# annikabrundyn/driving-dirty

Measured on AMD Instinct MI355X. Metric: 6-view scenes/sec fwd+bwd, roadmap model bs=32, higher is better.
Workload: dtype f32

## Files before the change

driving-dirty_amd/csrc/conv3x3.hip:

```cpp
#include <stdlib.h>

#include "dd_common.h"

namespace {

constexpr int EPI_BIAS_RELU_BITS = 5;
constexpr int EPI_RELU_BITS = 6;
constexpr int EPI_BIAS_STATS = 7;
constexpr int EPI_RELU_MASK_AFF = 8;
constexpr int EPI_RELU_BITS_W1 = 9;


template <int CIN, int S>
struct StripCfg {
  static constexpr int PXB = CIN * 4;
  static constexpr int CHUNKS = CIN / 4;
  static constexpr int NPX = 32 * S + 2;
  static constexpr int SLOTB = NPX * PXB;
  static constexpr int NCH = NPX * CHUNKS;
  static constexpr int NLOAD = (NCH + 63) / 64;
  static constexpr int SPILLB = (NLOAD * 64 - NCH) * 16;
  static constexpr int WAVEB = 3 * SLOTB + SPILLB;
  static constexpr int KGROUPS = (CIN == 32) ? 36 : 5;
  static constexpr int WFLOATS = KGROUPS * 64 * 4;
// ... 66 lines not shown
    v.z = in ? fmaxf(v.z * sc.z + sh.z, 0.f) : 0.f;
    v.w = in ? fmaxf(v.w * sc.w + sh.w, 0.f) : 0.f;
    *(f32x4*)dst = v;
  }
}

template <int CIN, int S, int EPI, int WPB, bool AFF = false>
__global__ __launch_bounds__(WPB * 64) void conv_strip_fwd(const float* __restrict__ x, const float* __restrict__ wp,
                                                           const float* __restrict__ bias,
                                                           const float* __restrict__ msk, float* __restrict__ y,
                                                           unsigned* __restrict__ bits_out, int B, int H, int W, int Ho,
                                                           int Wo, int nstrips, const float* __restrict__ aff = nullptr,
                                                           float* __restrict__ stats = nullptr) {
  using C = StripCfg<CIN, S>;
  extern __shared__ __attribute__((aligned(16))) char smem[];
  const int tid = threadIdx.x;
  const int lane = tid & 63;
  const int wave = __builtin_amdgcn_readfirstlane(tid >> 6);
  {
    f32x4* wl4 = (f32x4*)smem;
    const f32x4* wg4 = (const f32x4*)wp;
    for (int i = tid; i < C::WFLOATS / 4; i += WPB * 64) wl4[i] = wg4[i];
  }
  __syncthreads();
  char* ring = smem + C::WFLOATS * 4 + wave * C::WAVEB;
  char* spill = ring + 3 * C::SLOTB;
  const char* wl = smem;
  const int h = lane >> 5, n = lane & 31;
  const float bv = (EPI == DD_EPI_BIAS || EPI == DD_EPI_BIAS_RELU || EPI == EPI_BIAS_RELU_BITS || EPI == EPI_BIAS_STATS) ? bias[n] : 0.f;
  f32x4 asc = {1.f, 1.f, 1.f, 1.f}, ash = {0.f, 0.f, 0.f, 0.f};
  if (AFF) {
    asc = *(const f32x4*)(aff + 4 * (lane & 7));
    ash = *(const f32x4*)(aff + 32 + 4 * (lane & 7));
  }
  const float msc = (EPI == EPI_RELU_MASK_AFF) ? aff[64 + n] : 1.f, msh = (EPI == EPI_RELU_MASK_AFF) ? aff[96 + n] : 0.f;
  float st_sum = 0.f, st_sq = 0.f;

  long idx, end;
  dd_range((long)B * nstrips * Ho, blockIdx.x * WPB + wave, gridDim.x * WPB, idx, end);
  while (idx < end) {
    const long col = idx / Ho;
    const int y0 = (int)(idx - col * Ho);
    const int y1 = (int)min((long)Ho, y0 + (end - idx));
    idx += y1 - y0;
    const int b = (int)(col / nstrips), x0 = (int)(col % nstrips) * 32;
    const float* xb = x + (long)b * H * W * CIN;
    const int gx0 = S * x0 - 1;

#pragma unroll
    for (int d = 0; d < 3; ++d) {
      f32x4 t[C::NLOAD];
      const int iy = S * y0 - 1 + d;
      load_row<CIN, S>(xb, H, W, iy, gx0, lane, t);
      if constexpr (AFF) store_row_aff<S, true>(ring + ((iy + 1) % 3) * C::SLOTB, spill, lane, t, iy >= 0 && iy < H, gx0, W, asc, ash);
      else store_row<CIN, S, true>(ring + ((iy + 1) % 3) * C::SLOTB, spill, lane, t);
    }

    for (int yy = y0; yy < y1; ++yy) {
      f32x4 pre[S][C::NLOAD];
#pragma unroll
      for (int s = 0; s < S; ++s) load_row<CIN, S>(xb, H, W, S * yy + 2 + s, gx0, lane, pre[s]);

      const long orow = ((long)(b * Ho + yy) * Wo) * 32;
      float mreg[16];
      if (EPI == DD_EPI_RELU_MASK || EPI == EPI_RELU_MASK_AFF) {
        const __amdgpu_buffer_rsrc_t ms = dd_rsrc(msk + orow, Wo * 128);
#pragma unroll
        for (int r = 0; r < 16; ++r) mreg[r] = dd_bload1<DD_AUX_NT>(ms, ((x0 + dd_acc_row(r, lane)) * 32 + n) * 4);
      }
      if (EPI == EPI_RELU_BITS) {
        const __amdgpu_buffer_rsrc_t ms = dd_rsrc((const unsigned*)msk + (long)(b * Ho + yy) * Wo, Wo * 4);
#pragma unroll
        for (int r = 0; r < 16; ++r) mreg[r] = dd_bload1<DD_AUX_NT>(ms, (x0 + dd_acc_row(r, lane)) * 4);
      }
      __builtin_amdgcn_sched_barrier(0);

      f32x16 acc;
#pragma unroll
      for (int r = 0; r < 16; ++r) acc[r] = 0.f;

      if (CIN == 32) {
#pragma unroll
        for (int dy = 0; dy < 3; ++dy) {
          const char* rowb = ring + ((S * yy + dy) % 3) * C::SLOTB;
#pragma unroll
          for (int dx = 0; dx < 3; ++dx) {
            const int q = S * n + dx;
            const char* pa = rowb + q * 128;
            const int sw = swz<32>(q);
#pragma unroll
            for (int j = 0; j < 4; ++j) {
              const f32x4 a = *(const f32x4*)(pa + (((2 * j + h) ^ sw) << 4));
              const f32x4 w = *(const f32x4*)(wl + (((dy * 3 + dx) * 4 + j) * 64 + lane) * 16);
              acc = DD_MFMA(a.x, w.x, acc);
              acc = DD_MFMA(a.y, w.y, acc);
              acc = DD_MFMA(a.z, w.z, acc);
              acc = DD_MFMA(a.w, w.w, acc);
            }
          }
        }
      } else {
#pragma unroll
        for (int jp = 0; jp < 5; ++jp) {
          const int tap = min(2 * jp + h, 8);
          const int dy = tap / 3, dx = tap - 3 * dy;
          const char* rowb = ring + ((S * yy + dy) % 3) * C::SLOTB;
          const f32x4 a = *(const f32x4*)(rowb + (S * n + dx) * 16);
          const f32x4 w = *(const f32x4*)(wl + (jp * 64 + lane) * 16);
          acc = DD_MFMA(a.x, w.x, acc);
          acc = DD_MFMA(a.y, w.y, acc);
          acc = DD_MFMA(a.z, w.z, acc);
        }
      }

#pragma unroll
      for (int s = 0; s < S; ++s) {
        const int iy = S * yy + 2 + s;
        if constexpr (AFF) store_row_aff<S, true>(ring + ((iy + 1) % 3) * C::SLOTB, spill, lane, pre[s], iy >= 0 && iy < H, gx0, W, asc, ash);
        else store_row<CIN, S, true>(ring + ((iy + 1) % 3) * C::SLOTB, spill, lane, pre[s]);
      }

      const __amdgpu_buffer_rsrc_t ys = dd_rsrc(y + orow, Wo * 128);
      unsigned sign_word = 0;
#pragma unroll
      for (int r = 0; r < 16; ++r) {
        float v = acc[r];
        if (EPI == DD_EPI_BIAS || EPI == EPI_BIAS_STATS) v += bv;
        if (EPI == EPI_BIAS_STATS && x0 + dd_acc_row(r, lane) < Wo) {
          st_sum += v;
          st_sq += v * v;
        }
        if (EPI == DD_EPI_BIAS_RELU || EPI == EPI_BIAS_RELU_BITS) v = fmaxf(v + bv, 0.f);
        if (EPI == DD_EPI_RELU_MASK) v = (mreg[r] > 0.f) ? v : 0.f;
        if (EPI == EPI_RELU_MASK_AFF) v = (mreg[r] * msc + msh > 0.f) ? v : 0.f;
        if (EPI == EPI_RELU_BITS) v = ((__builtin_bit_cast(unsigned, mreg[r]) >> n) & 1u) ? v : 0.f;
        dd_bstore1<DD_AUX_NT>(ys, ((x0 + dd_acc_row(r, lane)) * 32 + n) * 4, v);
        if (EPI == EPI_BIAS_RELU_BITS) {
          const unsigned long long m = __ballot(v > 0.f);
          const int i0 = (r & 3) + 8 * (r >> 2);
          if (n == i0) sign_word = (unsigned)m;
          if (n == i0 + 4) sign_word = (unsigned)(m >> 32);
        }
      }
      if (EPI == EPI_BIAS_RELU_BITS) {
        const __amdgpu_buffer_rsrc_t bs = dd_rsrc(bits_out + (long)(b * Ho + yy) * Wo, Wo * 4);
        __builtin_amdgcn_raw_buffer_store_b32(sign_word, bs, (h == 0) ? (x0 + n) * 4 : -16, 0, 0);
      }
    }
  }
  if (EPI == EPI_BIAS_STATS) {
    const long gwl = ((long)(blockIdx.x * WPB + wave) * 64 + lane) * 2;
    stats[gwl] = st_sum;
    stats[gwl + 1] = st_sq;
  }
}

template <int WPB, int MASK>
__global__ __launch_bounds__(WPB * 64) void conv_s2_dgrad(const float* __restrict__ dy, const float* __restrict__ wp,
                                                          const float* __restrict__ msk, float* __restrict__ dx,
                                                          int B, int H, int W, int Ho, int Wo, int nstrips,
                                                          const float* __restrict__ aff = nullptr) {
  using C = StripCfg<32, 1>;
  extern __shared__ __attribute__((aligned(16))) char smem[];
  const int tid = threadIdx.x;
  const int lane = tid & 63;
  const int wave = __builtin_amdgcn_readfirstlane(tid >> 6);
  {
    f32x4* wl4 = (f32x4*)smem;
    const f32x4* wg4 = (const f32x4*)wp;
    for (int i = tid; i < C::WFLOATS / 4; i += WPB * 64) wl4[i] = wg4[i];
  }
  __syncthreads();
  const int nr = (H + 1) / 2;
  const float msc = (MASK == 3) ? aff[64 + (lane & 31)] : 1.f, msh = (MASK == 3) ? aff[96 + (lane & 31)] : 0.f;
  char* ring = smem + C::WFLOATS * 4 + wave * C::WAVEB;
  char* spill = ring + 3 * C::SLOTB;
  const char* wl = smem;
  const int h = lane >> 5, n = lane & 31;

  long idx, end;
  dd_range((long)B * nstrips * nr, blockIdx.x * WPB + wave, gridDim.x * WPB, idx, end);
  while (idx < end) {
    const long col = idx / nr;
    const int r0 = (int)(idx - col * nr);
    const int r1 = (int)min((long)nr, r0 + (end - idx));
    idx += r1 - r0;
    const int b = (int)(col / nstrips), s0 = (int)(col % nstrips) * 32;
    const float* dyb = dy + (long)b * Ho * Wo * 32;

#pragma unroll
    for (int d = 0; d < 2; ++d) {
      f32x4 t[C::NLOAD];
      load_row<32, 1>(dyb, Ho, Wo, r0 + d, s0, lane, t);
      store_row<32, 1, true>(ring + ((r0 + d) % 3) * C::SLOTB, spill, lane, t);
    }

    for (int r = r0; r < r1; ++r) {
      f32x4 pre[C::NLOAD];
      load_row<32, 1>(dyb, Ho, Wo, r + 2, s0, lane, pre);
      __builtin_amdgcn_sched_barrier(0);

      const char* row_r = ring + (r % 3) * C::SLOTB;
      const char* row_r1 = ring + ((r + 1) % 3) * C::SLOTB;
#define DD_TILE(PY, PX, NTAP, ...)                                                              \
  {                                                                                             \
    constexpr int taps[NTAP][3] = {__VA_ARGS__};                                                \
    const int yi = 2 * r + (PY);                                                                \
    const long orow = ((long)(b * H + min(yi, H - 1)) * W) * 32;                                \
    const int obytes = (yi < H) ? W * 128 : 0;                                                  \
    float mreg[16];                                                                             \
    if (MASK == 1 || MASK == 3) {                                                               \
      const __amdgpu_buffer_rsrc_t ms = dd_rsrc(msk + orow, obytes);                            \
      _Pragma("unroll") for (int rr = 0; rr < 16; ++rr)                                         \
        mreg[rr] = dd_bload1<DD_AUX_NT>(ms, ((2 * (s0 + dd_acc_row(rr, lane)) + (PX)) * 32 + n) * 4); \
      __builtin_amdgcn_sched_barrier(0);                                                        \
    }                                                                                           \
    if (MASK == 2) {                                                                            \
      const __amdgpu_buffer_rsrc_t ms = dd_rsrc((const unsigned*)msk + (long)(b * H + min(yi, H - 1)) * W, obytes / 32); \
      _Pragma("unroll") for (int rr = 0; rr < 16; ++rr)                                         \
        mreg[rr] = dd_bload1<DD_AUX_NT>(ms, (2 * (s0 + dd_acc_row(rr, lane)) + (PX)) * 4);      \
      __builtin_amdgcn_sched_barrier(0);                                                        \
    }                                                                                           \
    f32x16 acc;                                                                                 \
    _Pragma("unroll") for (int i = 0; i < 16; ++i) acc[i] = 0.f;                                \
    _Pragma("unroll") for (int t = 0; t < NTAP; ++t) {                                          \
      const char* rowp = taps[t][0] ? row_r1 : row_r;                                           \
      const int q = n + taps[t][1];                                                             \
      const char* pa = rowp + q * 128;                                                          \
      const int sw = swz<32>(q);                                                                \
      _Pragma("unroll") for (int j = 0; j < 4; ++j) {                                           \
        const f32x4 a = *(const f32x4*)(pa + (((2 * j + h) ^ sw) << 4));                        \
        const f32x4 w = *(const f32x4*)(wl + ((taps[t][2] * 4 + j) * 64 + lane) * 16);          \
        acc = DD_MFMA(a.x, w.x, acc);                                                           \
        acc = DD_MFMA(a.y, w.y, acc);                                                           \
        acc = DD_MFMA(a.z, w.z, acc);                                                           \
        acc = DD_MFMA(a.w, w.w, acc);                                                           \
      }                                                                                         \
    }                                                                                           \
    const __amdgpu_buffer_rsrc_t os = dd_rsrc(dx + orow, obytes);                               \
    _Pragma("unroll") for (int rr = 0; rr < 16; ++rr) {                                         \
      float v = acc[rr];                                                                        \
      if (MASK == 1) v = (mreg[rr] > 0.f) ? v : 0.f;                                            \
      if (MASK == 3) v = (mreg[rr] * msc + msh > 0.f) ? v : 0.f;                                \
      if (MASK == 2) v = ((__builtin_bit_cast(unsigned, mreg[rr]) >> n) & 1u) ? v : 0.f;        \
      dd_bstore1<DD_AUX_NT>(os, ((2 * (s0 + dd_acc_row(rr, lane)) + (PX)) * 32 + n) * 4, v);    \
    }                                                                                           \
  }
      DD_TILE(1, 1, 4, {1, 1, 0}, {1, 0, 2}, {0, 1, 6}, {0, 0, 8})
      store_row<32, 1, true>(ring + ((r + 2) % 3) * C::SLOTB, spill, lane, pre);
      DD_TILE(0, 1, 2, {0, 1, 3}, {0, 0, 5})
      DD_TILE(1, 0, 2, {1, 0, 1}, {0, 0, 7})
      DD_TILE(0, 0, 1, {0, 0, 4})
#undef DD_TILE
    }
  }
}

template <int CIN, int S, int WPB, bool AFF = false>
__global__ __launch_bounds__(WPB * 64) void conv_wgrad(const float* __restrict__ x, const float* __restrict__ dy,
                                                       float* __restrict__ part, float* __restrict__ bpart, int B,
                                                       int H, int W, int Ho, int Wo, int nstrips,
                                                       const float* __restrict__ aff = nullptr) {
  using C = StripCfg<CIN, S>;
  constexpr int NT = (CIN == 32) ? 9 : 1;
  extern __shared__ __attribute__((aligned(16))) char smem[];
  const int tid = threadIdx.x;
  const int lane = tid & 63;
  const int wave = __builtin_amdgcn_readfirstlane(tid >> 6);
  char* ring = smem + wave * C::WAVEB;
  char* spill = ring + 3 * C::SLOTB;
  const int h = lane >> 5, n = lane & 31;
  const int gw = blockIdx.x * WPB + wave;
  f32x4 asc = {1.f, 1.f, 1.f, 1.f}, ash = {0.f, 0.f, 0.f, 0.f};
  if (AFF) {
    asc = *(const f32x4*)(aff + 4 * (lane & 7));
    ash = *(const f32x4*)(aff + 32 + 4 * (lane & 7));
  }

  f32x16 acc[NT];
#pragma unroll
  for (int t = 0; t < NT; ++t)
#pragma unroll
    for (int r = 0; r < 16; ++r) acc[t][r] = 0.f;
  float bsum = 0.f;

  const int tap4 = min(n / 3, 8), c4 = n % 3;
  const int dy4 = tap4 / 3, dx4 = tap4 - 3 * dy4;

  long idx, end;
  dd_range((long)B * nstrips * Ho, gw, gridDim.x * WPB, idx, end);
  while (idx < end) {
    const long col = idx / Ho;
    const int y0 = (int)(idx - col * Ho);
    const int y1 = (int)min((long)Ho, y0 + (end - idx));
    idx += y1 - y0;
    const int b = (int)(col / nstrips), x0 = (int)(col % nstrips) * 32;
    const float* xb = x + (long)b * H * W * CIN;
    const float* dyb = dy + (long)b * Ho * Wo * 32;
    const int gx0 = S * x0 - 1;
    const int aoff = ((x0 + h) * 32 + n) * 4;

#pragma unroll
    for (int d = 0; d < 3; ++d) {
      f32x4 t[C::NLOAD];
      const int iy = S * y0 - 1 + d;
      load_row<CIN, S>(xb, H, W, iy, gx0, lane, t);
// ... 1342 lines not shown
      for (int c = 0; c < W2R_CHUNKS; ++c) t += tv[u][c];
      t = t * ((u == 1 || u == 2) ? 0.5f : 1.f) * ((v == 1 || v == 2) ? 0.5f : 1.f);
      z[0] += (u < 3 ? 1.f : 0.f) * t;
      z[1] += (u == 1 ? 1.f : u == 2 ? -1.f : 0.f) * t;
      z[2] += (u > 0 ? 1.f : 0.f) * t;
    }
#pragma unroll
    for (int ky = 0; ky < 3; ++ky) {
      out[ky][0] += (v < 3 ? 1.f : 0.f) * z[ky];
      out[ky][1] += (v == 1 ? 1.f : v == 2 ? -1.f : 0.f) * z[ky];
      out[ky][2] += (v > 0 ? 1.f : 0.f) * z[ky];
    }
  }
  const int o = dd_acc_row(r, l), jj = l & 31;
  float* dst = dw + ((long)o * 32 + jj) * 9;
#pragma unroll
  for (int a = 0; a < 9; ++a) dst[a] = out[a / 3][a % 3];
}

__global__ __launch_bounds__(1024) void conv_wino_wgrad_reduce(const float* __restrict__ part, const float* __restrict__ bpart,
                                                               float* __restrict__ dw, float* __restrict__ db, int nw) {
  constexpr int G = 16;
  __shared__ float red[4][G][64];
  const int l = threadIdx.x & 63, g = threadIdx.x >> 6;
  const int row = blockIdx.x;
  if (row == 48) {
    float s0 = 0.f;
    for (int w = g; w < nw; w += G) s0 += bpart[(long)w * 64 + l];
    red[0][g][l] = s0;
    __syncthreads();
    if (g != 0) return;
    float s = 0.f;
#pragma unroll
    for (int i = 0; i < G; ++i) s += red[0][i][l];
    const float other = __shfl_xor(s, 32);
    if (l < 32) db[l] = s + other;
    return;
  }
  const int ky = row >> 4, r = row & 15;
  float s[4] = {0.f, 0.f, 0.f, 0.f};
  for (int w = g; w < nw; w += G) {
#pragma unroll
    for (int p = 0; p < 4; ++p) s[p] += part[((((long)w * 3 + ky) * 4 + p) * 16 + r) * 64 + l];
  }
#pragma unroll
  for (int p = 0; p < 4; ++p) red[p][g][l] = s[p];
  __syncthreads();
  if (g != 0) return;
  float t[4] = {0.f, 0.f, 0.f, 0.f};
#pragma unroll
  for (int p = 0; p < 4; ++p)
#pragma unroll
    for (int i = 0; i < G; ++i) t[p] += red[p][i][l];
  const int o = dd_acc_row(r, l), j = l & 31;
  float* out = dw + ((long)o * 32 + j) * 9 + ky * 3;
  out[0] = (t[0] + t[1]) + t[2];
  out[1] = t[1] - t[2];
  out[2] = (t[1] + t[2]) + t[3];
}

__global__ void conv_wino_pack_kernel(const float* __restrict__ w, float* __restrict__ p, int kind) {
  const int idx = blockIdx.x * blockDim.x + threadIdx.x;
  if (idx >= WINO_UFLOATS) return;
  const int j = idx & 3, lane = (idx >> 2) & 63, g = (idx >> 8) & 1, hf = (idx >> 9) & 1, pos = (idx >> 10) & 3, ky = idx >> 12;
  const int co = (lane & 15) + 16 * hf, ci = 8 * (lane >> 4) + 4 * g + j;
  float t[3];
#pragma unroll
  for (int kx = 0; kx < 3; ++kx)
    t[kx] = kind == 0 ? w[((long)co * 32 + ci) * 9 + ky * 3 + kx] : w[((long)ci * 32 + co) * 9 + (2 - ky) * 3 + (2 - kx)];
  float u;
  if (pos == 0) u = t[0];
  else if (pos == 1) u = 0.5f * ((t[0] + t[1]) + t[2]);
  else if (pos == 2) u = 0.5f * ((t[0] - t[1]) + t[2]);
  else u = t[2];
  p[idx] = u;
}

__global__ __launch_bounds__(256) void relu_sign_bits_kernel(const float* __restrict__ x, unsigned* __restrict__ bits, long npix) {
  const int lane = threadIdx.x & 63;
  const long wave = ((long)blockIdx.x * blockDim.x + threadIdx.x) >> 6, nwaves = ((long)gridDim.x * blockDim.x) >> 6;
  for (long p0 = wave * 64; p0 < npix; p0 += nwaves * 64) {
    unsigned word = 0;
#pragma unroll 8
    for (int i = 0; i < 32; ++i) {
      const long p = p0 + 2 * i + (lane >> 5);
      const float v = p < npix ? x[p * 32 + (lane & 31)] : 0.f;
      const unsigned long long m = __ballot(v > 0.f);
      if (lane == 2 * i) word = (unsigned)m;
      if (lane == 2 * i + 1) word = (unsigned)(m >> 32);
    }
    if (p0 + lane < npix) bits[p0 + lane] = word;
  }
}

__global__ __launch_bounds__(256) void relu_bwd_pad_bits_kernel(const float* __restrict__ dy, const unsigned* __restrict__ bits_pad,
                                                                f32x4* __restrict__ out_pad, int B, int H, int W, int dy_cstore, int dy_coff) {
  const long total = (long)B * (H + 2) * (W + 2) * 8;
  for (long i = (long)blockIdx.x * blockDim.x + threadIdx.x; i < total; i += (long)gridDim.x * blockDim.x) {
    const int q = (int)(i & 7);
    const long pp = i >> 3;
    const int xx = (int)(pp % (W + 2)), yy = (int)((pp / (W + 2)) % (H + 2));
    const long b = pp / ((long)(W + 2) * (H + 2));
    f32x4 o = {0.f, 0.f, 0.f, 0.f};
    if (xx >= 1 && xx <= W && yy >= 1 && yy <= H) {
      const f32x4 g = *(const f32x4*)(dy + ((b * H + (yy - 1)) * W + (xx - 1)) * dy_cstore + dy_coff + 4 * q);
      const unsigned m = bits_pad[pp] >> (4 * q);
      o.x = (m & 1u) ? g.x : 0.f;
      o.y = (m & 2u) ? g.y : 0.f;
      o.z = (m & 4u) ? g.z : 0.f;
      o.w = (m & 8u) ? g.w : 0.f;
    }
    __builtin_nontemporal_store(o, out_pad + i);
  }
}

__global__ void relu_bwd_kernel(const f32x4* __restrict__ dy, const f32x4* __restrict__ y, f32x4* __restrict__ out,
                                long n4) {
  for (long i = (long)blockIdx.x * blockDim.x + threadIdx.x; i < n4; i += (long)gridDim.x * blockDim.x) {
    const f32x4 g = dy[i], v = y[i];
    f32x4 o;
    o.x = v.x > 0.f ? g.x : 0.f;
    o.y = v.y > 0.f ? g.y : 0.f;
    o.z = v.z > 0.f ? g.z : 0.f;
    o.w = v.w > 0.f ? g.w : 0.f;
    out[i] = o;
  }
}

int check_desc(const dd_conv_desc* d) {
  DD_REQUIRE(d != nullptr, DD_ERR_BAD_ARG, "conv: NULL descriptor");
  DD_REQUIRE(d->batch > 0 && d->height > 0 && d->width > 0, DD_ERR_BAD_ARG, "conv: non-positive size");
  DD_REQUIRE(d->ksize == 3 && d->pad == 1, DD_ERR_UNSUPPORTED, "conv: only k3 p1 is implemented (got k%d p%d)", d->ksize, d->pad);
  DD_REQUIRE(d->stride == 1 || d->stride == 2, DD_ERR_UNSUPPORTED, "conv: stride %d", d->stride);
  DD_REQUIRE(d->cout == 32, DD_ERR_UNSUPPORTED, "conv: Cout %d (only 32)", d->cout);
  DD_REQUIRE((d->cin_real == 32 && d->cin_store == 32) || (d->cin_real == 3 && d->cin_store == 4), DD_ERR_UNSUPPORTED,
             "conv: Cin %d stored as %d (supported: 32/32, 3/4)", d->cin_real, d->cin_store);
  DD_REQUIRE(!(d->cin_real == 3 && d->stride == 2), DD_ERR_UNSUPPORTED, "conv: Cin 3 with stride 2");
  DD_REQUIRE((long)d->width * 128 < (1L << 31), DD_ERR_UNSUPPORTED, "conv: row too long for a 32-bit buffer descriptor");
  return 0;
}

int resident_grid(const dd_conv_desc* d, long row_tiles, int wpb, int per_cu) {
  long blocks = (long)dd_cu_budget_internal() * per_cu;
  if (d->rows_per_task > 0) blocks = min(blocks, max(1L, row_tiles / d->rows_per_task / wpb));
  return (int)max(1L, min(blocks, (row_tiles + wpb - 1) / wpb));
}

template <int CIN, int S, int EPI, int WPB, bool AFF = false>
int launch_fwd(const float* x, const float* wp, const float* bias, const float* msk, float* y, const dd_conv_desc* d,
               hipStream_t st, unsigned* bits_out = nullptr, const float* aff = nullptr, float* stats = nullptr) {
  using C = StripCfg<CIN, S>;
  const int Ho = dd_conv_out(d->height, S), Wo = dd_conv_out(d->width, S);
  const int nstrips = (Wo + 31) / 32;
  const size_t lds = C::WFLOATS * 4 + (size_t)WPB * C::WAVEB;
  const int per_cu = (int)max((size_t)1, min((size_t)2, (size_t)(160 * 1024) / lds));
  const int grid = resident_grid(d, (long)d->batch * nstrips * Ho, WPB, per_cu);
  auto k = conv_strip_fwd<CIN, S, EPI, WPB, AFF>;
  if (int rc = dd_allow_lds((const void*)k, lds)) return rc;
  hipLaunchKernelGGL(k, dim3(grid), dim3(WPB * 64), lds, st, x, wp, bias, msk, y, bits_out, d->batch, d->height, d->width,
                     Ho, Wo, nstrips, aff, stats);
  DD_LAUNCH_CHECK("conv_strip_fwd");
  return 0;
}

template <int MASK>
int launch_s2_dgrad(const float* dy, const float* packed_dgrad, const float* relu_src, float* dx, const dd_conv_desc* d, hipStream_t st,
                    const float* aff) {
  using C = StripCfg<32, 1>;
  constexpr int WPB = 8;
  const int H = d->height, W = d->width, Ho = dd_conv_out(H, 2), Wo = dd_conv_out(W, 2);
  const int ns = (W + 1) / 2, nr = (H + 1) / 2;
  const int nstrips = (ns + 31) / 32;
  const size_t lds = C::WFLOATS * 4 + (size_t)WPB * C::WAVEB;
  const int grid = resident_grid(d, (long)d->batch * nstrips * nr, WPB, 1);
  auto k = conv_s2_dgrad<WPB, MASK>;
  if (int rc = dd_allow_lds((const void*)k, lds)) return rc;
  hipLaunchKernelGGL(k, dim3(grid), dim3(WPB * 64), lds, st, dy, packed_dgrad, relu_src, dx, d->batch, H, W, Ho, Wo, nstrips, aff);
  DD_LAUNCH_CHECK("conv_s2_dgrad");
  return 0;
}

template <int EPI>
int launch_wino2(const float* x, const float* up, const float* bias, const unsigned* bits_in, float* y, unsigned* bits_out,
                 const dd_conv_desc* d, hipStream_t st, const float* x4 = nullptr, float* w1part = nullptr, int* nw_out = nullptr) {
  using C = StripCfg<32, 1>;
  using C4 = StripCfg<4, 1>;
  constexpr int WPB = 4;
  const int nstrips = (d->width + 31) / 32;
  static const bool ring_env = getenv("DD_WINO2_RING") != nullptr;
  static const bool ring_w1 = getenv("DD_WINO2_RING_W1") != nullptr;
  const bool ring = ring_env || (EPI == EPI_RELU_BITS_W1 && ring_w1);
  DD_REQUIRE((long)d->height * d->width * 128 < (1L << 30), DD_ERR_UNSUPPORTED, "conv_wino2: image of %d x %d pixels: the kernel addresses an image with 30-bit offsets",
             d->height, d->width);
  const size_t lds = (size_t)WINO2_UFLOATS * 4 + (ring ? (size_t)WPB * (4 * C::SLOTB + C::SPILLB) : 0) +
                     (EPI == EPI_RELU_BITS_W1 ? (size_t)WPB * (4 * C4::SLOTB + C4::SPILLB) + 128 : 0);
  const int grid = resident_grid(d, (long)d->batch * nstrips * ((d->height + 1) / 2), WPB, 1);
  if (nw_out) *nw_out = grid * WPB;
  if (int rc = dd_allow_lds(ring ? (const void*)conv_wino2_fwd<EPI, WPB> : (const void*)conv_wino2r_fwd<EPI, WPB>, lds)) return rc;
  constexpr int pf_rows = 1;
  auto kring = conv_wino2_fwd<EPI, WPB>;
  auto kreg = conv_wino2r_fwd<EPI, WPB>;
  if (ring) hipLaunchKernelGGL(kring, dim3(grid), dim3(WPB * 64), lds, st, x, up, bias, bits_in, y, bits_out, d->batch, d->height, d->width, nstrips, x4, w1part);
  else hipLaunchKernelGGL(kreg, dim3(grid), dim3(WPB * 64), lds, st, x, up, bias, bits_in, y, bits_out, d->batch, d->height, d->width, nstrips, x4, w1part, pf_rows);
  DD_LAUNCH_CHECK("conv_wino2_fwd");
  return 0;
}

template <int EPI>
int launch_wino(const float* x, const float* up, const float* bias, const unsigned* bits_in, float* y, unsigned* bits_out,
                const dd_conv_desc* d, hipStream_t st) {
  using C = StripCfg<32, 1>;
  constexpr int WPB = 8;
  const int nstrips = (d->width + 31) / 32;
  const size_t lds = (size_t)WINO_UFLOATS * 4 + (size_t)WPB * C::WAVEB;
  const int grid = resident_grid(d, (long)d->batch * nstrips * d->height, WPB, 1);
  auto k = conv_wino_fwd<EPI, WPB>;
  if (int rc = dd_allow_lds((const void*)k, lds)) return rc;
  hipLaunchKernelGGL(k, dim3(grid), dim3(WPB * 64), lds, st, x, up, bias, bits_in, y, bits_out, d->batch, d->height, d->width, nstrips);
  DD_LAUNCH_CHECK("conv_wino_fwd");
  return 0;
}

}

extern "C" {

int64_t dd_conv_packed_floats(const dd_conv_desc* d, int32_t kind) {
  if (check_desc(d)) return -1;
  if (kind != 0 && d->cin_real != 32) return -1;
  return d->cin_real == 32 ? 36 * 64 * 4 : 5 * 64 * 4;
}

int dd_conv_pack(const float* w_oihw, float* packed, const dd_conv_desc* d, int32_t kind, void* stream) {
  if (int rc = check_desc(d)) return rc;
  DD_REQUIRE(w_oihw && packed, DD_ERR_BAD_ARG, "conv_pack: NULL pointer");
  DD_REQUIRE(kind >= 0 && kind <= 2, DD_ERR_BAD_ARG, "conv_pack: kind %d", kind);
  DD_REQUIRE(kind == 0 || d->cin_real == 32, DD_ERR_UNSUPPORTED, "conv_pack: dgrad packing needs Cin 32");
  const int n = d->cin_real == 32 ? 36 * 64 * 4 : 5 * 64 * 4;
  hipLaunchKernelGGL(conv_pack_kernel, dim3((n + 255) / 256), dim3(256), 0, (hipStream_t)stream, w_oihw, packed,
                     d->cin_real, kind);
  DD_LAUNCH_CHECK("conv_pack");
  return 0;
}

int dd_conv_fwd(const float* x, const float* packed_fwd, const float* bias, const float* mask, float* y,
                const dd_conv_desc* d, int32_t epilogue, void* stream) {
  if (int rc = check_desc(d)) return rc;
  DD_REQUIRE(x && packed_fwd && y, DD_ERR_BAD_ARG, "conv_fwd: NULL pointer");
  DD_REQUIRE(epilogue != DD_EPI_RELU_MASK || mask, DD_ERR_BAD_ARG, "conv_fwd: RELU_MASK epilogue needs a mask");
  DD_REQUIRE((epilogue != DD_EPI_BIAS && epilogue != DD_EPI_BIAS_RELU) || bias, DD_ERR_BAD_ARG, "conv_fwd: bias epilogue needs a bias");
  hipStream_t st = (hipStream_t)stream;
#define DD_DISPATCH(CIN, S, WPB)                                                                                    \
  switch (epilogue) {                                                                                               \
    case DD_EPI_NONE: return launch_fwd<CIN, S, DD_EPI_NONE, WPB>(x, packed_fwd, bias, mask, y, d, st);             \
    case DD_EPI_BIAS: return launch_fwd<CIN, S, DD_EPI_BIAS, WPB>(x, packed_fwd, bias, mask, y, d, st);             \
    case DD_EPI_BIAS_RELU: return launch_fwd<CIN, S, DD_EPI_BIAS_RELU, WPB>(x, packed_fwd, bias, mask, y, d, st);   \
    case DD_EPI_RELU_MASK: return launch_fwd<CIN, S, DD_EPI_RELU_MASK, WPB>(x, packed_fwd, bias, mask, y, d, st);   \
    default: return dd_fail(DD_ERR_BAD_ARG, "conv_fwd: epilogue %d", epilogue);                                     \
  }
  if (d->cin_store == 4) { DD_DISPATCH(4, 1, 8) }
  if (d->stride == 1) { DD_DISPATCH(32, 1, 8) }
  DD_DISPATCH(32, 2, 4)
#undef DD_DISPATCH
}

int dd_conv_fwd_relu_bits(const float* x, const float* packed_fwd, const float* bias, float* y, uint32_t* relu_bits,
                          const dd_conv_desc* d, void* stream) {
  if (int rc = check_desc(d)) return rc;
  DD_REQUIRE(x && packed_fwd && bias && y && relu_bits, DD_ERR_BAD_ARG, "conv_fwd_relu_bits: NULL pointer");
  hipStream_t st = (hipStream_t)stream;
  if (d->cin_store == 4) return launch_fwd<4, 1, EPI_BIAS_RELU_BITS, 8>(x, packed_fwd, bias, nullptr, y, d, st, relu_bits);
  if (d->stride == 1) return launch_fwd<32, 1, EPI_BIAS_RELU_BITS, 8>(x, packed_fwd, bias, nullptr, y, d, st, relu_bits);
  return launch_fwd<32, 2, EPI_BIAS_RELU_BITS, 4>(x, packed_fwd, bias, nullptr, y, d, st, relu_bits);
}

static int conv_dgrad_impl(const float* dy, const float* packed_dgrad, const float* relu_src, int mask_mode, float* dx,
                           const dd_conv_desc* d, void* stream, const float* aff = nullptr);

int dd_conv_dgrad(const float* dy, const float* packed_dgrad, const float* relu_src, float* dx, const dd_conv_desc* d,
                  void* stream) {
  return conv_dgrad_impl(dy, packed_dgrad, relu_src, relu_src ? 1 : 0, dx, d, stream);
}

int dd_conv_dgrad_relu_bits(const float* dy, const float* packed_dgrad, const uint32_t* relu_bits, float* dx,
                            const dd_conv_desc* d, void* stream) {
  DD_REQUIRE(relu_bits, DD_ERR_BAD_ARG, "conv_dgrad_relu_bits: NULL mask");
  return conv_dgrad_impl(dy, packed_dgrad, (const float*)relu_bits, 2, dx, d, stream);
}

int dd_conv_dgrad_bn(const float* dy, const float* packed_dgrad, const float* pre_bn, const float* affine, float* dx,
                     const dd_conv_desc* d, void* stream) {
  DD_REQUIRE(pre_bn && affine, DD_ERR_BAD_ARG, "conv_dgrad_bn: NULL mask / affine");
  return conv_dgrad_impl(dy, packed_dgrad, pre_bn, 3, dx, d, stream, affine);
}

static int conv_dgrad_impl(const float* dy, const float* packed_dgrad, const float* relu_src, int mask_mode, float* dx,
                           const dd_conv_desc* d, void* stream, const float* aff) {
  if (int rc = check_desc(d)) return rc;
  DD_REQUIRE(dy && packed_dgrad && dx, DD_ERR_BAD_ARG, "conv_dgrad: NULL pointer");
  DD_REQUIRE(d->cin_real == 32, DD_ERR_UNSUPPORTED, "conv_dgrad: Cin %d (the first layer has no data gradient)", d->cin_real);
  hipStream_t st = (hipStream_t)stream;
  if (d->stride == 1) {
    if (mask_mode == 3) return launch_fwd<32, 1, EPI_RELU_MASK_AFF, 8>(dy, packed_dgrad, nullptr, relu_src, dx, d, st, nullptr, aff);
    if (mask_mode == 2) return launch_fwd<32, 1, EPI_RELU_BITS, 8>(dy, packed_dgrad, nullptr, relu_src, dx, d, st);
    return mask_mode ? launch_fwd<32, 1, DD_EPI_RELU_MASK, 8>(dy, packed_dgrad, nullptr, relu_src, dx, d, st)
                     : launch_fwd<32, 1, DD_EPI_NONE, 8>(dy, packed_dgrad, nullptr, nullptr, dx, d, st);
// ... 299 lines not shown
```

Measured before the change: 4341.

## Add register-resident, software-pipelined stride-2 conv forward kernel with ReLU sign bits

Adds a specialized stride-2, 32-channel forward conv kernel for the bias+ReLU+sign-bits epilogue. Weights are held in registers instead of LDS, input rows are kept in a three-slot LDS ring, and the next rows' global loads and the previous row's output and bit stores are interleaved with the MFMA chain. Sign words are built with writelane instead of a select. It trades higher register pressure and one block per CU for less LDS traffic and better load/compute overlap, and only applies when the input fits the 32-bit offset bound.

```diff
diff --git a/driving-dirty_amd/csrc/conv3x3.hip b/driving-dirty_amd/csrc/conv3x3.hip
--- a/driving-dirty_amd/csrc/conv3x3.hip
+++ b/driving-dirty_amd/csrc/conv3x3.hip
@@ -242,6 +242,156 @@
     const long gwl = ((long)(blockIdx.x * WPB + wave) * 64 + lane) * 2;
     stats[gwl] = st_sum;
     stats[gwl + 1] = st_sq;
+  }
+}
+
+template <int V>
+struct IntC {
+  static constexpr int value = V;
+};
+
+constexpr int S2F_SLOTB = StripCfg<32, 2>::SLOTB + StripCfg<32, 2>::SPILLB;
+constexpr int S2F_FAR = 1 << 30;
+
+template <int WPB>
+__global__ __launch_bounds__(WPB * 64) void conv_s2_fwd_bits(const float* __restrict__ x, const float* __restrict__ wp,
+                                                             const float* __restrict__ bias, float* __restrict__ y,
+                                                             unsigned* __restrict__ bits_out, int B, int H, int W, int Ho, int Wo,
+                                                             int nstrips) {
+  using C = StripCfg<32, 2>;
+  constexpr int SLOT = S2F_SLOTB, FAR = S2F_FAR;
+  constexpr int D = 3;
+  extern __shared__ __attribute__((aligned(16))) char smem[];
+  const int lane = threadIdx.x & 63;
+  const int wave = __builtin_amdgcn_readfirstlane(threadIdx.x >> 6);
+  const int h = lane >> 5, n = lane & 31;
+  char* ring = smem + wave * 3 * SLOT;
+  f32x4 wr[36];
+#pragma unroll
+  for (int g = 0; g < 36; ++g) wr[g] = ((const f32x4*)wp)[g * 64 + lane];
+  const float bv = bias[n];
+  const char* abase[3][4];
+#pragma unroll
+  for (int dx = 0; dx < 3; ++dx)
+#pragma unroll
+    for (int j = 0; j < 4; ++j) {
+      const int q = 2 * n + dx;
+      abase[dx][j] = ring + q * 128 + (((2 * j + h) ^ swz<32>(q)) << 4);
+    }
+  char* wbase[C::NLOAD];
+#pragma unroll
+  for (int i = 0; i < C::NLOAD; ++i) {
+    const int c = lane + 64 * i, q = c >> 3, ch = c & 7;
+    wbase[i] = ring + q * 128 + ((ch ^ swz<32>(q)) << 4);
+  }
+
+  long idx, end;
+  dd_range((long)B * nstrips * Ho, blockIdx.x * WPB + wave, gridDim.x * WPB, idx, end);
+  while (idx < end) {
+    const long col = idx / Ho;
+    const int y0 = (int)(idx - col * Ho);
+    const int y1 = (int)min((long)Ho, y0 + (end - idx));
+    idx += y1 - y0;
+    const int b = (int)(col / nstrips), x0 = (int)(col % nstrips) * 32;
+    const float* xb = x + (long)b * H * W * 32;
+    float* yb = y + (long)b * Ho * Wo * 32;
+    unsigned* bb = bits_out + (long)b * Ho * Wo;
+    const int pitch = W * 128, opitch = Wo * 128, bpitch = Wo * 4;
+    const int gx0 = 2 * x0 - 1;
+    const int q0 = gx0 + (lane >> 3), lo1 = (q0 + 8) * 128 + (lane & 7) * 16;
+    const int lo0 = (q0 >= 0) ? lo1 - 1024 : FAR, lo8 = (lane + 512 < C::NCH) ? lo1 + 7 * 1024 : FAR;
+    auto xchunk = [&](__amdgpu_buffer_rsrc_t rs, int so, int i) {
+      return i == 0 ? dd_bload4<DD_AUX_NT>(rs, lo0, so) : i == 8 ? dd_bload4<DD_AUX_NT>(rs, lo8, so) : dd_bload4<DD_AUX_NT>(rs, lo1, so + (i - 1) * 1024);
+    };
+    const int yo = ((x0 + 4 * h) * 32 + n) * 4;
+    const int bo = (h == 0) ? (x0 + n) * 4 : FAR;
+
+    auto xload = [&](int iy, f32x4 (&r)[C::NLOAD]) {
+      const bool ok = (iy >= 0) && (iy < H);
+      const int so = ok ? iy * pitch : 0;
+      const __amdgpu_buffer_rsrc_t rs = dd_rsrc(xb, ok ? so + pitch : 0);
+#pragma unroll
+      for (int i = 0; i < C::NLOAD; ++i) r[i] = xchunk(rs, so, i);
+    };
+    float pend[16];
+    unsigned psign = 0;
+    int prow = -1;
+#pragma unroll
+    for (int r = 0; r < 16; ++r) pend[r] = 0.f;
+    auto ystore = [&](int r) {
+      const __amdgpu_buffer_rsrc_t ys = dd_rsrc(yb, (prow + 1) * opitch);
+      dd_bstore<DD_AUX_NT>(ys, yo, pend[r], prow * opitch + ((r & 3) + 8 * (r >> 2)) * 128);
+    };
+    auto bstore = [&]() {
+      const __amdgpu_buffer_rsrc_t bs = dd_rsrc(bb, (prow + 1) * bpitch);
+      __builtin_amdgcn_raw_buffer_store_b32(psign, bs, bo, prow * bpitch, 0);
+    };
+
+    int ph = (2 * y0) % 3;
+#pragma unroll
+    for (int d = 0; d < 3; ++d) {
+      f32x4 t[C::NLOAD];
+      xload(2 * y0 - 1 + d, t);
+      const int slot = (ph + d) % 3;
+#pragma unroll
+      for (int i = 0; i < C::NLOAD; ++i) *(f32x4*)(wbase[i] + slot * SLOT) = t[i];
+    }
+    f32x4 aq[D];
+#pragma unroll
+    for (int g = 0; g < D; ++g) aq[g] = *(const f32x4*)(abase[0][g] + ph * SLOT);
+
+    auto row = [&](auto phase, int yy) {
+      constexpr int P = decltype(phase)::value;
+      f32x4 pre0[C::NLOAD], pre1[C::NLOAD];
+      const int iy0 = 2 * yy + 2, iy1 = 2 * yy + 3;
+      const int so0 = (iy0 < H) ? iy0 * pitch : 0, so1 = (iy1 < H) ? iy1 * pitch : 0;
+      const __amdgpu_buffer_rsrc_t rs0 = dd_rsrc(xb, (iy0 < H) ? so0 + pitch : 0), rs1 = dd_rsrc(xb, (iy1 < H) ? so1 + pitch : 0);
+      f32x16 acc;
+#pragma unroll
+      for (int r = 0; r < 16; ++r) acc[r] = 0.f;
+#pragma unroll
+      for (int g = 0; g < 36; ++g) {
+        __builtin_amdgcn_sched_barrier(0);
+        const int gn = g + D;
+        const f32x4 an = (gn < 36) ? *(const f32x4*)(abase[(gn >> 2) % 3][gn & 3] + ((P + gn / 12) % 3) * SLOT)
+                                   : *(const f32x4*)(abase[0][gn - 36] + ((P + 2) % 3) * SLOT);
+        if (g < 9) pre0[g] = xchunk(rs0, so0, g);
+        if (g >= 12 && g < 21) pre1[g - 12] = xchunk(rs1, so1, g - 12);
+        if (g >= 9 && g < 25) ystore(g - 9);
+        if (g == 25) bstore();
+        if (g >= 12 && g < 21) *(f32x4*)(wbase[g - 12] + P * SLOT) = pre0[g - 12];
+        if (g >= 24 && g < 33) *(f32x4*)(wbase[g - 24] + ((P + 1) % 3) * SLOT) = pre1[g - 24];
+        const f32x4 a = aq[g % D], w = wr[g];
+        acc = DD_MFMA(a.x, w.x, acc);
+        acc = DD_MFMA(a.y, w.y, acc);
+        acc = DD_MFMA(a.z, w.z, acc);
+        acc = DD_MFMA(a.w, w.w, acc);
+        aq[g % D] = an;
+      }
+      __builtin_amdgcn_sched_barrier(0);
+      unsigned sw = 0;
+#pragma unroll
+      for (int r = 0; r < 16; ++r) {
+        const float v = fmaxf(acc[r] + bv, 0.f);
+        pend[r] = v;
+        const unsigned long long m = __ballot(v > 0.f);
+        const int i0 = (r & 3) + 8 * (r >> 2);
+        asm("v_writelane_b32 %0, %1, %2" : "+v"(sw) : "s"((unsigned)m), "n"(i0));
+        asm("v_writelane_b32 %0, %1, %2" : "+v"(sw) : "s"((unsigned)(m >> 32)), "n"(i0 + 4));
+      }
+      psign = sw;
+      prow = yy;
+    };
+
+    for (int yy = y0; yy < y1; ++yy) {
+      if (ph == 0) row(IntC<0>{}, yy);
+      else if (ph == 1) row(IntC<1>{}, yy);
+      else row(IntC<2>{}, yy);
+      ph = (ph == 0) ? 2 : ph - 1;
+    }
+#pragma unroll
+    for (int r = 0; r < 16; ++r) ystore(r);
+    bstore();
   }
 }
 
@@ -1890,6 +2040,17 @@
   using C = StripCfg<CIN, S>;
   const int Ho = dd_conv_out(d->height, S), Wo = dd_conv_out(d->width, S);
   const int nstrips = (Wo + 31) / 32;
+  if constexpr (CIN == 32 && S == 2 && EPI == EPI_BIAS_RELU_BITS && !AFF) {
+    if ((long)d->height * d->width * 128 < (long)S2F_FAR) {
+      const size_t lds2 = (size_t)WPB * 3 * S2F_SLOTB;
+      const int grid2 = resident_grid(d, (long)d->batch * nstrips * Ho, WPB, 1);
+      auto k2 = conv_s2_fwd_bits<WPB>;
+      if (int rc = dd_allow_lds((const void*)k2, lds2)) return rc;
+      hipLaunchKernelGGL(k2, dim3(grid2), dim3(WPB * 64), lds2, st, x, wp, bias, y, bits_out, d->batch, d->height, d->width, Ho, Wo, nstrips);
+      DD_LAUNCH_CHECK("conv_s2_fwd_bits");
+      return 0;
+    }
+  }
   const size_t lds = C::WFLOATS * 4 + (size_t)WPB * C::WAVEB;
   const int per_cu = (int)max((size_t)1, min((size_t)2, (size_t)(160 * 1024) / lds));
   const int grid = resident_grid(d, (long)d->batch * nstrips * Ho, WPB, per_cu);
```

Result: no change. 4334 (median of 2 runs) (-0.2%).
